# renaudbedard/raytracing-in-one-weekend

Hardware: AMD Instinct MI355X
Metric: Msamples/s, 486-sphere cover scene 1920x1080 8-bounce (higher is better)
Workload: dtype f32

## Files before the change

### include/rtow.h

```cpp
#ifndef RTOW_H
#define RTOW_H

#include <stddef.h>
#include <stdint.h>

#ifdef __cplusplus
extern "C" {
#endif

#if defined(_WIN32)
#define RTOW_API __declspec(dllexport)
#else
#define RTOW_API __attribute__((visibility("default")))
#endif

#define RTOW_API_VERSION 12

typedef enum RtowResult {
    RTOW_SUCCESS = 0,
    RTOW_ERROR_INVALID_VALUE = 1,
    RTOW_ERROR_MEMORY_ALLOCATION = 2,
    RTOW_ERROR_NO_DEVICE = 3,
    RTOW_ERROR_NO_SCENE = 4,
    RTOW_ERROR_UNSUPPORTED = 5,
// ... 102 lines not shown
    int32_t sceneInLds;
    uint64_t sceneBytesDevice;
    uint64_t hitSpillBytes;
    int32_t hitListCapacity;
    int32_t wideCodes;
    int32_t thresholdSet;
    int32_t schedulerTune[9];
} RtowSceneInfo;


typedef struct RtowView {
    RtowFloat3 origin;
    RtowFloat3 lowerLeftCorner;
    RtowFloat3 horizontal, vertical;
    RtowFloat3 forward, up, right;
    float lensRadius;
} RtowView;

typedef enum RtowRngPolicy { RTOW_RNG_REFERENCE = 0, RTOW_RNG_PER_SAMPLE = 1, RTOW_RNG_PER_SAMPLE_XOROSHIRO = 2 } RtowRngPolicy;

typedef enum RtowCubemapChannelType { RTOW_CUBEMAP_UNSIGNED_BYTE = 0, RTOW_CUBEMAP_SIGNED_HALF = 1 } RtowCubemapChannelType;
typedef struct RtowCubemapDesc {
    int32_t faceWidth, faceHeight;
    int32_t channelType;
    int32_t pixelStride;
    const void* faces;
} RtowCubemapDesc;

typedef struct RtowBlueNoiseDesc {
    uint32_t rowStride, textureCount;
    const void* texels;
} RtowBlueNoiseDesc;
typedef struct RtowStbNoiseDesc {
    uint32_t rowStride, textureCount;
    const void* scalar;
    const void* vector2;
    const void* cosineUnitVector3;
    const void* unitVector2;
    const void* unitVector3;
} RtowStbNoiseDesc;

typedef struct RtowEnvironment {
    int32_t skyType;
    RtowFloat3 skyBottomColor;
    RtowFloat3 skyTopColor;
} RtowEnvironment;

typedef struct RtowSampleParams {
    RtowFloat2 size;
    int32_t sliceOffset;
    int32_t sliceDivider;
    uint32_t seed;
    RtowView view;
    RtowEnvironment environment;
    uint32_t sampleCountRange[2];
    int32_t traceDepth;
    int32_t subPixelJitter;
    int32_t noiseColor;
    RtowFloat2 sampleCountWeightExtrema;
    int32_t diagnosticsStride;
    int32_t noiseTextureIndex;
    int32_t rngPolicy;
} RtowSampleParams;

typedef struct RtowAccumBuffers {
    float* color;
    float* normal;
    float* albedo;
    float* sampleCountWeight;
} RtowAccumBuffers;

typedef struct RtowContext_t* RtowContext;

typedef void (*RtowLogCallback)(int32_t level, const char* tag, const char* message, void* userData);

typedef enum RtowContextFlags {
    RTOW_CONTEXT_EXACT_TIES_ALWAYS = 1u << 0,
    RTOW_CONTEXT_EXACT_TIES_NEVER = 1u << 1,
    RTOW_CONTEXT_REFERENCE_DIAGNOSTICS = 1u << 2,
    RTOW_CONTEXT_NO_CAMERA_RAY_LISTS = 1u << 3,
    RTOW_CONTEXT_NO_CHUNK_ORDER = 1u << 4,
    RTOW_CONTEXT_FORCE_WIDE_CODES = 1u << 5,
    RTOW_CONTEXT_NO_CHAIN_FUSION = 1u << 7,
    RTOW_CONTEXT_NO_THRESHOLD_TUNING = 1u << 6
} RtowContextFlags;

typedef struct RtowContextOptions {
    int32_t deviceOrdinal;
    RtowLogCallback logCallback;
    void* logCallbackData;
    int32_t logCallbackLevel;
    uint32_t flags;
    int32_t ldsSceneBudgetBytes;
    int32_t schedulerTune[9];
    int32_t hitListCapacity;
    int32_t sliceBlockThreads;
} RtowContextOptions;

RTOW_API int rtowGetApiVersion(void);
RTOW_API const char* rtowErrorString(int result);

RTOW_API int rtowCreateContext(const RtowContextOptions* options, RtowContext* outContext);
RTOW_API int rtowDestroyContext(RtowContext context);

RTOW_API int rtowUploadScene(RtowContext context, const RtowSceneDesc* scene);
RTOW_API int rtowGetSceneInfo(RtowContext context, RtowSceneInfo* outInfo);

RTOW_API int rtowUploadSkyCubemap(RtowContext context, const RtowCubemapDesc* cubemap);

RTOW_API int rtowUploadBlueNoise(RtowContext context, const RtowBlueNoiseDesc* noise);
RTOW_API int rtowUploadStbNoise(RtowContext context, const RtowStbNoiseDesc* noise);

RTOW_API int rtowSampleBatch(RtowContext context, const RtowSampleParams* params,
                             const RtowAccumBuffers* in, const RtowAccumBuffers* out,
                             void* diagnostics, const volatile uint8_t* cancel);

RTOW_API int rtowSampleBatchDevice(RtowContext context, const RtowSampleParams* params,
                                   const RtowAccumBuffers* in, const RtowAccumBuffers* out,
                                   void* diagnostics, void* stream, const volatile uint8_t* cancel);

RTOW_API int rtowSampleBatchChainDevice(RtowContext context, int32_t count, const RtowSampleParams* params ,
                                        const RtowAccumBuffers* in, const RtowAccumBuffers* out,
                                        void* const* diagnostics , void* stream, const volatile uint8_t* cancel);

typedef struct RtowAdaptiveFeed {
    const RtowFloat2* extremaIn;
    RtowFloat2* extremaOut;
    int32_t lag;
    int32_t reserved;
} RtowAdaptiveFeed;

RTOW_API int rtowSampleBatchChainAdaptiveDevice(RtowContext context, int32_t count, const RtowSampleParams* params ,
                                                const RtowAccumBuffers* in, const RtowAccumBuffers* out,
                                                void* const* diagnostics , const RtowAdaptiveFeed* feed,
                                                void* stream, const volatile uint8_t* cancel);

RTOW_API int rtowSampleBatchGroupDevice(RtowContext context, int32_t count, const RtowSampleParams* params ,
                                        const RtowAccumBuffers* in, const RtowAccumBuffers* outs ,
                                        void* const* diagnostics , void* stream, const volatile uint8_t* cancel);

RTOW_API int rtowSampleBatchChain(RtowContext context, int32_t count, const RtowSampleParams* params ,
                                  const RtowAccumBuffers* in, const RtowAccumBuffers* out,
                                  void* const* diagnostics , const volatile uint8_t* cancel);

RTOW_API int rtowRegisterHostBuffer(RtowContext context, void* pointer, size_t sizeInBytes);
RTOW_API int rtowUnregisterHostBuffer(RtowContext context, void* pointer);

RTOW_API int rtowProbeNearestHit(RtowContext context, const RtowFloat3* origin, const RtowFloat3* direction, float time, float* distance, int32_t* entityIndex);

typedef struct RtowRay {
    RtowFloat3 origin;  float time;
    RtowFloat3 direction; float pad;
} RtowRay;

typedef struct RtowHitBuffers {
    float*   distance;
    int32_t* entityIndex;
    float*   normal;
} RtowHitBuffers;

RTOW_API int rtowTraceRaysDevice(RtowContext context, int32_t count, const RtowRay* rays ,
                                 const RtowHitBuffers* hits, void* stream);

typedef struct RtowTraceViewParams {
    int32_t width, height;
    RtowView view;
// ... 102 lines not shown
```

### raytracing-in-one-weekend_amd/abi.py

```python
import ctypes as C

RTOW_API_VERSION = 12

RTOW_SUCCESS = 0
RTOW_ERROR_INVALID_VALUE = 1
RTOW_ERROR_MEMORY_ALLOCATION = 2
RTOW_ERROR_NO_DEVICE = 3
RTOW_ERROR_NO_SCENE = 4
RTOW_ERROR_UNSUPPORTED = 5
RTOW_ERROR_LAUNCH_FAILURE = 6
RTOW_ERROR_CANCELLED = 7
RTOW_ERROR_CAPACITY = 8
RTOW_ERROR_INTERNAL = 99

ENTITY_NONE, ENTITY_SPHERE, ENTITY_RECT, ENTITY_BOX, ENTITY_TRIANGLE = range(5)
MATERIAL_STANDARD, MATERIAL_DIELECTRIC, MATERIAL_PROBABILISTIC_VOLUME = range(3)
TEXTURE_NONE, TEXTURE_CONSTANT, TEXTURE_CHECKER_PATTERN, TEXTURE_PERLIN_NOISE, TEXTURE_IMAGE, TEXTURE_CONSTANT_SCALAR = range(6)
SKY_NONE, SKY_GRADIENT, SKY_CUBEMAP = range(3)
NOISE_WHITE, NOISE_BLUE, NOISE_SPATIOTEMPORAL_BLUE = range(3)
MEMCPY_HOST_TO_HOST, MEMCPY_HOST_TO_DEVICE, MEMCPY_DEVICE_TO_HOST, MEMCPY_DEVICE_TO_DEVICE = range(4)


class Float2(C.Structure):
    _fields_ = [("x", C.c_float), ("y", C.c_float)]
# ... 18 lines not shown
                ("scalarValueChannel", C.c_int32), ("imageIndex", C.c_int32)]


class Image(C.Structure):
    _fields_ = [("width", C.c_int32), ("height", C.c_int32), ("pixelStride", C.c_int32), ("pixels", C.c_void_p)]


class Material(C.Structure):
    _fields_ = [("type", C.c_int32), ("albedo", Texture), ("glossiness", Texture), ("emission", Texture),
                ("metallic", Texture), ("parameter", C.c_float)]


class Entity(C.Structure):
    _fields_ = [("type", C.c_int32), ("moving", C.c_int32), ("rotation", Float4), ("position", Float3),
                ("destinationOffset", Float3), ("timeRange", Float2), ("materialIndex", C.c_int32),
                ("size", Float3), ("contentIndex", C.c_int32)]


class Triangle(C.Structure):
    _fields_ = [("data", Float3 * 3), ("normals", Float3 * 3), ("textureCoordinates", Float2 * 3)]


class SceneDesc(C.Structure):
    _fields_ = [("entities", C.POINTER(Entity)), ("entityCount", C.c_int32),
                ("materials", C.POINTER(Material)), ("materialCount", C.c_int32),
                ("maxBvhDepth", C.c_int32), ("triangles", C.POINTER(Triangle)), ("triangleCount", C.c_int32),
                ("images", C.POINTER(Image)), ("imageCount", C.c_int32)]


class SceneInfo(C.Structure):
    _fields_ = [("entityCount", C.c_int32), ("materialCount", C.c_int32), ("bvhNodeCount", C.c_int32),
                ("bvhDepth", C.c_int32), ("ldsBytesScene", C.c_int32), ("sceneInLds", C.c_int32),
                ("sceneBytesDevice", C.c_uint64), ("hitSpillBytes", C.c_uint64), ("hitListCapacity", C.c_int32), ("wideCodes", C.c_int32),
                ("thresholdSet", C.c_int32), ("schedulerTune", C.c_int32 * 9)]


class View(C.Structure):
    _fields_ = [("origin", Float3), ("lowerLeftCorner", Float3), ("horizontal", Float3), ("vertical", Float3),
                ("forward", Float3), ("up", Float3), ("right", Float3), ("lensRadius", C.c_float)]


CUBEMAP_UNSIGNED_BYTE, CUBEMAP_SIGNED_HALF = 0, 1
RNG_REFERENCE, RNG_PER_SAMPLE, RNG_PER_SAMPLE_XOROSHIRO = 0, 1, 2


class CubemapDesc(C.Structure):
    _fields_ = [("faceWidth", C.c_int32), ("faceHeight", C.c_int32), ("channelType", C.c_int32), ("pixelStride", C.c_int32),
                ("faces", C.c_void_p)]


class BlueNoiseDesc(C.Structure):
    _fields_ = [("rowStride", C.c_uint32), ("textureCount", C.c_uint32), ("texels", C.c_void_p)]


class StbNoiseDesc(C.Structure):
    _fields_ = [("rowStride", C.c_uint32), ("textureCount", C.c_uint32), ("scalar", C.c_void_p), ("vector2", C.c_void_p),
                ("cosineUnitVector3", C.c_void_p), ("unitVector2", C.c_void_p), ("unitVector3", C.c_void_p)]


class Environment(C.Structure):
    _fields_ = [("skyType", C.c_int32), ("skyBottomColor", Float3), ("skyTopColor", Float3)]


class SampleParams(C.Structure):
    _fields_ = [("size", Float2), ("sliceOffset", C.c_int32), ("sliceDivider", C.c_int32), ("seed", C.c_uint32),
                ("view", View), ("environment", Environment), ("sampleCountRange", C.c_uint32 * 2),
                ("traceDepth", C.c_int32), ("subPixelJitter", C.c_int32), ("noiseColor", C.c_int32),
                ("sampleCountWeightExtrema", Float2), ("diagnosticsStride", C.c_int32), ("noiseTextureIndex", C.c_int32),
                ("rngPolicy", C.c_int32)]


class AccumBuffers(C.Structure):
    _fields_ = [("color", C.c_void_p), ("normal", C.c_void_p), ("albedo", C.c_void_p),
                ("sampleCountWeight", C.c_void_p)]


class AdaptiveFeed(C.Structure):
    _fields_ = [("extremaIn", C.c_void_p), ("extremaOut", C.c_void_p), ("lag", C.c_int32), ("reserved", C.c_int32)]


LogCallback = C.CFUNCTYPE(None, C.c_int32, C.c_char_p, C.c_char_p, C.c_void_p)


CONTEXT_EXACT_TIES_ALWAYS, CONTEXT_EXACT_TIES_NEVER, CONTEXT_REFERENCE_DIAGNOSTICS, CONTEXT_NO_CAMERA_RAY_LISTS, CONTEXT_NO_CHUNK_ORDER, CONTEXT_FORCE_WIDE_CODES, CONTEXT_NO_THRESHOLD_TUNING, CONTEXT_NO_CHAIN_FUSION = 1, 2, 4, 8, 16, 32, 64, 128
GATHER_COLOR, GATHER_NORMAL, GATHER_ALBEDO, GATHER_SAMPLE_COUNT_WEIGHT, GATHER_ALL, GATHER_NO_BATCH_WAIT, GATHER_LOOPBACK = 1, 2, 4, 8, 15, 16, 32


class ContextOptions(C.Structure):
    _fields_ = [("deviceOrdinal", C.c_int32), ("logCallback", LogCallback), ("logCallbackData", C.c_void_p),
                ("logCallbackLevel", C.c_int32), ("flags", C.c_uint32), ("ldsSceneBudgetBytes", C.c_int32), ("schedulerTune", C.c_int32 * 9),
                ("hitListCapacity", C.c_int32), ("sliceBlockThreads", C.c_int32)]


class CommId(C.Structure):
    _fields_ = [("bytes", C.c_char * 128)]


class HybridPlan(C.Structure):
    _fields_ = [("tileCount", C.c_int32), ("groupCount", C.c_int32), ("tile", C.c_int32), ("group", C.c_int32),
                ("sliceOffset", C.c_int32), ("sliceDivider", C.c_int32), ("samples", C.c_uint32), ("seed", C.c_uint32)]


class Metrics(C.Structure):
    _fields_ = [("totalRayCount", C.c_int32), ("totalSamples", C.c_int32), ("sampleCountWeightExtrema", Float2),
                ("sampleCountExtrema", C.c_int32 * 2), ("totalRayCount64", C.c_int64), ("totalSamples64", C.c_int64)]


class CombineParams(C.Structure):
    _fields_ = [("width", C.c_int32), ("height", C.c_int32), ("debugMode", C.c_int32), ("ldrAlbedo", C.c_int32)]


RTOW_DENOISE_DEMODULATE_ALBEDO = 1
DENOISE_DEFAULT_ITERATIONS = 5
DENOISE_DEFAULT_NORMAL_SHARPNESS = 4
DENOISE_DEFAULT_COLOR_SIGMA = 0.5
DENOISE_DEFAULT_ALBEDO_SIGMA = 0.5
DENOISE_DEFAULT_FLAGS = RTOW_DENOISE_DEMODULATE_ALBEDO


class DenoiseParams(C.Structure):
    _fields_ = [("width", C.c_int32), ("height", C.c_int32), ("iterations", C.c_int32), ("normalSharpness", C.c_int32),
                ("colorSigma", C.c_float), ("albedoSigma", C.c_float), ("flags", C.c_int32), ("reserved", C.c_int32)]


class Ray(C.Structure):
    _fields_ = [("origin", Float3), ("time", C.c_float), ("direction", Float3), ("pad", C.c_float)]


RAY_DTYPE = [("origin", "<f4", (3,)), ("time", "<f4"), ("direction", "<f4", (3,)), ("pad", "<f4")]


class HitBuffers(C.Structure):
    _fields_ = [("distance", C.c_void_p), ("entityIndex", C.c_void_p), ("normal", C.c_void_p)]


class TraceViewParams(C.Structure):
    _fields_ = [("width", C.c_int32), ("height", C.c_int32), ("view", View), ("time", C.c_float), ("reserved", C.c_int32)]


def denoise_scratch_bytes(width, height):
    return int(width) * int(height) * 12


EXPORTED_SYMBOLS = [
    "rtowGetApiVersion", "rtowErrorString", "rtowCreateContext", "rtowDestroyContext", "rtowUploadScene",
    "rtowUploadSkyCubemap", "rtowUploadBlueNoise", "rtowUploadStbNoise", "rtowGetSceneInfo", "rtowSampleBatch", "rtowSampleBatchDevice", "rtowGetLastSampleKernelMs",
    "rtowReduceMetricsDevice", "rtowCombineDevice", "rtowFinalizeDevice", "rtowAddAccumDevice", "rtowDeviceAlloc", "rtowDeviceFree",
    "rtowDeviceCopy", "rtowDeviceMemset", "rtowSynchronize", "rtowGetBatchStatus", "rtowRegisterHostBuffer", "rtowUnregisterHostBuffer",
    "rtowSampleBatchChainDevice", "rtowSampleBatchChain", "rtowCommSetLibraryPath", "rtowCommGetUniqueId", "rtowCommInit", "rtowCommDestroy", "rtowGatherRowsDevice",
    "rtowHybridPlan", "rtowExchangeAccumDevice", "rtowSampleBatchGroupDevice",
    "rtowCombineFinalizeDevice", "rtowReduceMetricsDeviceAsync", "rtowProbeNearestHit", "rtowSampleBatchChainAdaptiveDevice",
    "rtowDenoiseDevice", "rtowTraceRaysDevice", "rtowTraceViewDevice",
]
```

### raytracing-in-one-weekend_amd/csrc/rtow_api.hip

```cpp
#include <hip/hip_runtime.h>

#include <algorithm>
#include <atomic>
#include <cfloat>
#include <chrono>
#include <cstdio>
#include <cstring>
#include <mutex>
#include <string>
#include <thread>
#include <vector>

#include "../../include/rtow.h"
#include "rtow_context.h"

#ifndef RTOW_GROUP_SLOT_BLOCK
#define RTOW_GROUP_SLOT_BLOCK 4
#endif
static constexpr unsigned kGroupSlotBlock = RTOW_GROUP_SLOT_BLOCK;
#ifndef RTOW_PIXEL_GATE
#define RTOW_PIXEL_GATE 1
#endif
#ifndef RTOW_URGENT_RAYS_PER_SAMPLE
#define RTOW_URGENT_RAYS_PER_SAMPLE 18.0f
// ... 852 lines not shown
    void* pinnedDevice = nullptr;
    ok = ok && hipHostGetDevicePointer(&pinnedDevice, pinned, 0) == hipSuccess;
    if (!ok) { if (pinned) (void)hipHostFree(pinned); rtowDestroyContext(ctx); return RTOW_ERROR_MEMORY_ALLOCATION; }
    ctx->hCancel = (volatile uint32_t*)pinned;
    ctx->hMetricsRecord = (volatile RtowMetrics*)((uint8_t*)pinned + 64);
    ctx->dMetricsRecord = (RtowMetrics*)((uint8_t*)pinnedDevice + 64);
    ctx->hCancel[0] = 0u;
    ctx->hCancel[1] = 0u;
    ctx->hCancel[2] = 0u;
    ctx->hCancel[3] = 0u;
    logf(ctx, 4, "rtow", "context on device %d (%s, %d CUs)", ordinal, prop.gcnArchName, ctx->cuCount);
    if (ctx->flags & RTOW_CONTEXT_NO_CHAIN_FUSION) {
        ctx->chainFusion = false;
    } else {
        unsigned pairs = 0, stale = 0, timeouts = 0;
        hipError_t le = hipSuccess;
        for (int attempt = 0; attempt < 2; attempt++) {
            le = runXcdCoherenceLitmus(ctx->cuCount, ctx->stream, &pairs, &stale, &timeouts);
            if (le != hipSuccess || stale != 0 || (pairs > 0 && timeouts == 0)) break;
            logf(ctx, 3, "rtow", "same-XCD hand-over litmus inconclusive (%u pairs, %u timeouts): %s", pairs, timeouts, attempt == 0 ? "once more" : "giving up");
        }
        ctx->chainFusion = le == hipSuccess && pairs > 0 && stale == 0 && timeouts == 0;
        if (le != hipSuccess) (void)hipGetLastError();
        logf(ctx, ctx->chainFusion ? 4 : 3, "rtow", "same-XCD hand-over litmus: %u pairs, %u stale dwords, %u timeouts%s", pairs, stale, timeouts,
             ctx->chainFusion ? "" : stale ? " - unsafe here: chained batches will run one launch per batch" : " - inconclusive: chained batches will run one launch per batch");
    }
    *outContext = ctx;
    return RTOW_SUCCESS;
}

RTOW_API int rtowDestroyContext(RtowContext ctx)
{
    if (!ctx) return RTOW_ERROR_INVALID_VALUE;
    (void)hipSetDevice(ctx->device);
    if (ctx->stream) (void)hipStreamSynchronize(ctx->stream);
    if (ctx->dScene) (void)hipFree(ctx->dScene);
    if (ctx->dEntityOfPrim) (void)hipFree(ctx->dEntityOfPrim);
    if (ctx->dWorkCounter) (void)hipFree(ctx->dWorkCounter);
    if (ctx->dChunkCost) { (void)hipFree(ctx->dChunkCost); (void)hipFree(ctx->dChunkOrder); (void)hipFree(ctx->dPixelCost); (void)hipFree(ctx->dTicketMap); }
    if (ctx->dChunkDone) (void)hipFree(ctx->dChunkDone);
    if (ctx->dXcdState) (void)hipFree(ctx->dXcdState);
    if (ctx->dChainBatches) (void)hipFree(ctx->dChainBatches);
    if (ctx->dPixCand) (void)hipFree(ctx->dPixCand);
    if (ctx->dCubemap) (void)hipFree(ctx->dCubemap);
    if (ctx->dBlueNoise) (void)hipFree(ctx->dBlueNoise);
    if (ctx->dStbNoise) (void)hipFree(ctx->dStbNoise);
    if (ctx->dTexBlob) (void)hipFree(ctx->dTexBlob);
    if (ctx->dRefTree) (void)hipFree(ctx->dRefTree);
    if (ctx->dHitSpill) (void)hipFree(ctx->dHitSpill);
    if (ctx->dUnitRecords) (void)hipFree(ctx->dUnitRecords);
    if (ctx->dPartials) (void)hipFree(ctx->dPartials);
    if (ctx->dExtremaPartials) (void)hipFree(ctx->dExtremaPartials);
    if (ctx->dExtremaKeys) (void)hipFree(ctx->dExtremaKeys);
    if (ctx->dByteThresholds) (void)hipFree(ctx->dByteThresholds);
    dropThresholdTuning(ctx);
    if (ctx->dProbeSink) (void)hipFree(ctx->dProbeSink);
    if (ctx->dTieRedo) (void)hipFree(ctx->dTieRedo);
    if (ctx->dTieBits) (void)hipFree(ctx->dTieBits);
    if (ctx->dTieInputs) (void)hipFree(ctx->dTieInputs);
    if (ctx->dHistSpill) (void)hipFree(ctx->dHistSpill);
    if (ctx->dRedoSpill) (void)hipFree(ctx->dRedoSpill);
    if (ctx->hCancel) (void)hipHostFree((void*)ctx->hCancel);
    if (ctx->dColor) { (void)hipFree(ctx->dColor); (void)hipFree(ctx->dNormal); (void)hipFree(ctx->dAlbedo); (void)hipFree(ctx->dScw); }
    if (ctx->dDiag) (void)hipFree(ctx->dDiag);
    releaseComm(ctx);
    for (const RtowContext_t::HostRange& r : ctx->hostRanges) (void)hipHostUnregister(r.base);
    ctx->hostRanges.clear();
    if (ctx->evStart) (void)hipEventDestroy(ctx->evStart);
    if (ctx->evStop) (void)hipEventDestroy(ctx->evStop);
    if (ctx->evBatchDone) (void)hipEventDestroy(ctx->evBatchDone);
    if (ctx->evMetricsDone) (void)hipEventDestroy(ctx->evMetricsDone);
    if (ctx->stream) (void)hipStreamDestroy(ctx->stream);
    delete ctx;
    return RTOW_SUCCESS;
}

RTOW_API int rtowUploadScene(RtowContext ctx, const RtowSceneDesc* scene)
{
    if (!ctx || !scene) return RTOW_ERROR_INVALID_VALUE;
    std::lock_guard<std::mutex> lock(ctx->mu);
    HIP_TRY(ctx, hipSetDevice(ctx->device), RTOW_ERROR_NO_DEVICE);
    CompiledScene compiled;
    std::string err;
    const int rc = compileScene(scene, RTOW_STACK_CAPACITY, &compiled, &err);
    if (rc != RTOW_SUCCESS) {
        logf(ctx, 2, "scene", "%s", err.c_str());
        return rc;
    }
    HIP_TRY(ctx, hipDeviceSynchronize(), RTOW_ERROR_LAUNCH_FAILURE);
    RTOW_TRY(growDevice(ctx, ctx->dSceneCapacity, compiled.blob.size(), {devBuf(ctx->dScene, compiled.blob.size())}));
    HIP_TRY(ctx, hipMemcpy(ctx->dScene, compiled.blob.data(), compiled.blob.size(), hipMemcpyHostToDevice), RTOW_ERROR_LAUNCH_FAILURE);
    if (!compiled.entityOfPrim.empty()) {
        const size_t n = compiled.entityOfPrim.size();
        RTOW_TRY(growDevice(ctx, ctx->entityOfPrimCapacity, n, {devBuf(ctx->dEntityOfPrim, n * sizeof(int32_t))}));
        HIP_TRY(ctx, hipMemcpy(ctx->dEntityOfPrim, compiled.entityOfPrim.data(), n * sizeof(int32_t), hipMemcpyHostToDevice), RTOW_ERROR_LAUNCH_FAILURE);
    }
    if (!compiled.texBlob.empty()) {
        RTOW_TRY(growDevice(ctx, ctx->texBlobCapacity, compiled.texBlob.size(), {devBuf(ctx->dTexBlob, compiled.texBlob.size())}));
        HIP_TRY(ctx, hipMemcpy(ctx->dTexBlob, compiled.texBlob.data(), compiled.texBlob.size(), hipMemcpyHostToDevice), RTOW_ERROR_LAUNCH_FAILURE);
        compiled.texBlob.clear();
        compiled.texBlob.shrink_to_fit();
    }
    if (ctx->flags & RTOW_CONTEXT_REFERENCE_DIAGNOSTICS) {
        if (compiled.refTreeDepth > 62) { logf(ctx, 2, "scene", "RTOW_CONTEXT_REFERENCE_DIAGNOSTICS supports MaxBvhDepth <= 62"); return RTOW_ERROR_CAPACITY; }
        RTOW_TRY(growDevice(ctx, ctx->refTreeCapacity, compiled.refTree.size(), {devBuf(ctx->dRefTree, compiled.refTree.size())}));
        HIP_TRY(ctx, hipMemcpy(ctx->dRefTree, compiled.refTree.data(), compiled.refTree.size(), hipMemcpyHostToDevice), RTOW_ERROR_LAUNCH_FAILURE);
    }
    compiled.refTree.clear();
    compiled.refTree.shrink_to_fit();
    HIP_TRY(ctx, launchPrepareMaterials(ctx->dScene, compiled.layout, ctx->stream), RTOW_ERROR_LAUNCH_FAILURE);
    HIP_TRY(ctx, launchPrepareEntities(ctx->dScene, compiled.layout, ctx->stream), RTOW_ERROR_LAUNCH_FAILURE);
    HIP_TRY(ctx, hipStreamSynchronize(ctx->stream), RTOW_ERROR_LAUNCH_FAILURE);
    if (compiled.layout.sceneKind >= SCENE_KIND_GENERAL && compiled.entityCount > 0)
        HIP_TRY(ctx, hipMemcpy(compiled.blob.data() + compiled.layout.primOffset, ctx->dScene + compiled.layout.primOffset, (size_t)compiled.entityCount * sizeof(GpuPrim), hipMemcpyDeviceToHost),
                RTOW_ERROR_LAUNCH_FAILURE);
    if (ctx->flags & (RTOW_CONTEXT_EXACT_TIES_ALWAYS | RTOW_CONTEXT_EXACT_TIES_NEVER)) {
        const bool volumes = compiled.layout.sceneKind == SCENE_KIND_VOLUMES || compiled.layout.sceneKind == SCENE_KIND_VOLUMES_TEXTURED;
        if (!volumes) compiled.layout.exactTies = (ctx->flags & RTOW_CONTEXT_EXACT_TIES_ALWAYS) ? 1u : 0u;
    }
    {
        const int rc = sizeHitSpill(ctx, compiled.layout.sceneKind, compiled.layout.exactTies != 0, compiled.entityCount);
        if (rc != RTOW_SUCCESS) return rc;
    }
    const bool wide = compiled.entityCount > 65535 || compiled.layout.nodeCount > 65535u || (ctx->flags & RTOW_CONTEXT_FORCE_WIDE_CODES) != 0;
    ctx->wideCodes = wide;
    if (!ctx->userTune) {
        const int* base = kThresholdFamilies[compiled.layout.sceneKind <= SCENE_KIND_SPHERES_MOTION ? 0 : 1];
        for (int k = 0; k < 9; k++) ctx->tune[k] = base[k];
    } else if (ctx->userSliceDefault) {
        ctx->tune[8] = 16;
    }
    std::lock_guard<std::mutex> sceneLock(ctx->sceneMu);
    ctx->scene = std::move(compiled);
    ctx->ldsPlan = planLds(wide, ctx->scene.layout, 0u, ctx->ldsSceneBudget);
    ctx->ldsSceneBytes = ctx->ldsPlan.sceneBytes;
    ctx->ldsNodeCount = ctx->ldsPlan.nodeCount;
    ctx->haveScene = true;
    ctx->triWatchOff = false;
    ctx->hCancel[3] = 0u;
    ctx->sceneSerial++;
    ctx->orderValid = false;
    dropThresholdTuning(ctx);
    ctx->sppSinceUpload = 0;
    ctx->sceneSignatureNow = sceneSignature(ctx->scene, wide);
    if (!ctx->userTune && !(ctx->flags & RTOW_CONTEXT_NO_THRESHOLD_TUNING))
        for (const RtowContext_t::TuneCacheEntry& e : ctx->tuneCache)
            if (e.signature == ctx->sceneSignatureNow) {
                candidateThresholds(e.winner, ctx->tune, 8);
                ctx->tunedCandidate = e.winner;
                ctx->tunedScene = ctx->sceneSerial;
            }
    logf(ctx, 4, "scene", "%d entities, %u BVH nodes, depth %u, %u bytes (%u in LDS)%s", ctx->scene.entityCount, ctx->scene.layout.nodeCount,
         ctx->scene.layout.bvhDepth, ctx->scene.layout.totalBytes, ctx->ldsSceneBytes,
         ctx->scene.layout.exactTies ? ", exact-tie kernels" : "");
    return RTOW_SUCCESS;
}

RTOW_API int rtowUploadSkyCubemap(RtowContext ctx, const RtowCubemapDesc* cubemap)
{
    if (!ctx) return RTOW_ERROR_INVALID_VALUE;
    std::lock_guard<std::mutex> lock(ctx->mu);
    HIP_TRY(ctx, hipSetDevice(ctx->device), RTOW_ERROR_NO_DEVICE);
    if (!cubemap || !cubemap->faces) {
        HIP_TRY(ctx, hipDeviceSynchronize(), RTOW_ERROR_LAUNCH_FAILURE);
        if (ctx->dCubemap) (void)hipFree(ctx->dCubemap);
        ctx->dCubemap = nullptr;
        ctx->cubemapCapacity = 0;
// ... 483 lines not shown
```

### raytracing-in-one-weekend_amd/csrc/rtow_bvh.cpp

```cpp
#include "rtow_bvh.h"
#include "rtow_reforder.h"

#include <algorithm>
#include <cfloat>
#include <cmath>
#include <cstring>
#include <numeric>
#include <queue>

namespace rtow {

namespace {

struct Box {
    float lo[3], hi[3];
    void reset() { for (int a = 0; a < 3; a++) { lo[a] = FLT_MAX; hi[a] = -FLT_MAX; } }
    void grow(const Box& b) { for (int a = 0; a < 3; a++) { lo[a] = std::min(lo[a], b.lo[a]); hi[a] = std::max(hi[a], b.hi[a]); } }
    double area() const
    {
        const double dx = (double)hi[0] - lo[0], dy = (double)hi[1] - lo[1], dz = (double)hi[2] - lo[2];
        return 2.0 * (dx * dy + dy * dz + dz * dx);
    }
};

// ... 51 lines not shown

        const int self = (int)nodes.size();
        nodes.push_back(TmpNode{});
        Box b0, b1;
        const int c0 = build(idx, begin, begin + bestSplit, depthLeft - 1, depth + 1, &b0);
        const int c1 = build(idx, begin + bestSplit, end, depthLeft - 1, depth + 1, &b1);
        nodes[self].box[0] = b0; nodes[self].box[1] = b1;
        nodes[self].child[0] = c0; nodes[self].child[1] = c1;
        *outBox = b0;
        outBox->grow(b1);
        return self;
    }

    int buildBinned(std::vector<int>& idx, int begin, int end, int depthLeft, int depth, long long cap, Box* outBox)
    {
        const int n = end - begin;
        float clo[3] = {FLT_MAX, FLT_MAX, FLT_MAX}, chi[3] = {-FLT_MAX, -FLT_MAX, -FLT_MAX};
        for (int i = begin; i < end; i++)
            for (int a = 0; a < 3; a++) { const float c = centroid[a][idx[i]]; clo[a] = std::min(clo[a], c); chi[a] = std::max(chi[a], c); }
        double bestCost = DBL_MAX;
        int bestAxis = -1, bestBin = -1;
        for (int axis = 0; axis < 3; axis++) {
            const float ext = chi[axis] - clo[axis];
            if (!(ext > 0)) continue;
            const float scale = (float)kBins / ext;
            Box bb[kBins];
            int cnt[kBins] = {0};
            for (int b = 0; b < kBins; b++) bb[b].reset();
            for (int i = begin; i < end; i++) {
                int b = (int)((centroid[axis][idx[i]] - clo[axis]) * scale);
                b = b < 0 ? 0 : b >= kBins ? kBins - 1 : b;
                cnt[b]++;
                bb[b].grow(primBox[idx[i]]);
            }
            double rArea[kBins];
            int rCnt[kBins];
            Box acc;
            acc.reset();
            int c = 0;
            for (int b = kBins - 1; b >= 1; b--) { if (cnt[b]) acc.grow(bb[b]); c += cnt[b]; rArea[b] = c ? acc.area() : 0.0; rCnt[b] = c; }
            acc.reset();
            c = 0;
            for (int b = 1; b < kBins; b++) {
                if (cnt[b - 1]) acc.grow(bb[b - 1]);
                c += cnt[b - 1];
                if (c == 0 || rCnt[b] == 0 || c > cap || rCnt[b] > cap) continue;
                const double cost = acc.area() * c + rArea[b] * rCnt[b];
                if (cost < bestCost) { bestCost = cost; bestAxis = axis; bestBin = b; }
            }
        }
        int mid;
        if (bestAxis >= 0) {
            const float scale = (float)kBins / (chi[bestAxis] - clo[bestAxis]);
            const std::vector<float>& cc = centroid[bestAxis];
            const float lo = clo[bestAxis];
            const int bin = bestBin;
            int* first = idx.data() + begin;
            int* split = std::partition(first, idx.data() + end, [&](int p) {
                int b = (int)((cc[p] - lo) * scale);
                b = b < 0 ? 0 : b >= kBins ? kBins - 1 : b;
                return b < bin;
            });
            mid = begin + (int)(split - first);
        } else {
            int axis = 0;
            for (int a = 1; a < 3; a++) if (chi[a] - clo[a] > chi[axis] - clo[axis]) axis = a;
            const std::vector<float>& cc = centroid[axis];
            mid = begin + n / 2;
            std::nth_element(idx.begin() + begin, idx.begin() + mid, idx.begin() + end, [&cc](int a, int b) { return cc[a] < cc[b] || (cc[a] == cc[b] && a < b); });
        }
        const int self = (int)nodes.size();
        nodes.push_back(TmpNode{});
        Box b0, b1;
        const int c0 = build(idx, begin, mid, depthLeft - 1, depth + 1, &b0);
        const int c1 = build(idx, mid, end, depthLeft - 1, depth + 1, &b1);
        nodes[self].box[0] = b0; nodes[self].box[1] = b1;
        nodes[self].child[0] = c0; nodes[self].child[1] = c1;
        *outBox = b0;
        outBox->grow(b1);
        return self;
    }
};

float texColor(const RtowTexture& t, int c)
{
    switch (t.type) {
        case RTOW_TEXTURE_CONSTANT: return c == 0 ? t.mainColor.x : c == 1 ? t.mainColor.y : t.mainColor.z;
        case RTOW_TEXTURE_CONSTANT_SCALAR: return t.parameter;
    }
    return 0.0f;
}
float texScalar(const RtowTexture& t)
{
    switch (t.type) {
        case RTOW_TEXTURE_CONSTANT: return texColor(t, t.scalarValueChannel);
        case RTOW_TEXTURE_CONSTANT_SCALAR: return t.parameter;
    }
    return 0.0f;
}
bool texSupported(const RtowTexture& t)
{
    return t.type == RTOW_TEXTURE_NONE || t.type == RTOW_TEXTURE_CONSTANT || t.type == RTOW_TEXTURE_CONSTANT_SCALAR || t.type == RTOW_TEXTURE_IMAGE;
}
GpuTexture packTexture(const RtowTexture& t)
{
    GpuTexture g{};
    g.type = t.type;
    g.image = t.type == RTOW_TEXTURE_IMAGE ? t.imageIndex : -1;
    g.channel = t.scalarValueChannel;
    g.parameter = t.parameter;
    g.mainColor[0] = t.mainColor.x; g.mainColor[1] = t.mainColor.y; g.mainColor[2] = t.mainColor.z;
    return g;
}
bool almostOne(float v) { return std::fabs(1.0f - v) < 1e-6f; }

uint32_t align16(uint32_t v) { return (v + 15u) & ~15u; }

void setBoxes(GpuNode& g, const Box& b0, const Box& b1)
{
    g.lox[0] = b0.lo[0]; g.lox[1] = b1.lo[0]; g.loy[0] = b0.lo[1]; g.loy[1] = b1.lo[1]; g.loz[0] = b0.lo[2]; g.loz[1] = b1.lo[2];
    g.hix[0] = b0.hi[0]; g.hix[1] = b1.hi[0]; g.hiy[0] = b0.hi[1]; g.hiy[1] = b1.hi[1]; g.hiz[0] = b0.hi[2]; g.hiz[1] = b1.hi[2];
}

}

int compileScene(const RtowSceneDesc* desc, int maxDepth, CompiledScene* out, std::string* err)
{
    if (!desc || !out || !desc->entities || !desc->materials || desc->entityCount <= 0 || desc->materialCount <= 0) {
        *err = "null or empty scene description";
        return RTOW_ERROR_INVALID_VALUE;
    }
    const int n = desc->entityCount;
    if (n > (1 << 23) || desc->materialCount > 32767) {
        *err = "scene exceeds 8388608 entities or 32767 materials (30-bit hit codes / 32-bit blob offsets, 15-bit path-history codes)";
        return RTOW_ERROR_CAPACITY;
    }
    if (maxDepth <= 0) maxDepth = RTOW_DEFAULT_MAX_BVH_DEPTH;
    if (maxDepth > RTOW_STACK_CAPACITY) maxDepth = RTOW_STACK_CAPACITY;
    if ((1LL << std::min(maxDepth, 30)) < n) {
        *err = "maxBvhDepth too small for the entity count";
        return RTOW_ERROR_CAPACITY;
    }

    std::vector<GpuMaterial> mats(desc->materialCount);
    std::vector<uint32_t> matClass(desc->materialCount);
    bool hasVolumes = false, hasImageTextures = false;
    for (int i = 0; i < desc->materialCount; i++) {
        const RtowMaterial& m = desc->materials[i];
        if (m.type != RTOW_MATERIAL_STANDARD && m.type != RTOW_MATERIAL_DIELECTRIC && m.type != RTOW_MATERIAL_PROBABILISTIC_VOLUME) {
            *err = "unknown material type";
            return RTOW_ERROR_INVALID_VALUE;
        }
        hasVolumes |= m.type == RTOW_MATERIAL_PROBABILISTIC_VOLUME;
        if (!texSupported(m.albedo) || !texSupported(m.glossiness) || !texSupported(m.emission) || !texSupported(m.metallic)) {
            *err = "texture type not built (CheckerPattern / PerlinNoise are dead code in the reference)";
            return RTOW_ERROR_UNSUPPORTED;
        }
        bool textured = false;
        for (const RtowTexture* t : {&m.albedo, &m.glossiness, &m.emission, &m.metallic}) {
            if (t->type != RTOW_TEXTURE_IMAGE) continue;
            textured = true;
            if (t->imageIndex >= desc->imageCount || (t->imageIndex >= 0 && !desc->images)) {
                *err = "imageIndex out of range";
                return RTOW_ERROR_INVALID_VALUE;
            }
            if (t->scalarValueChannel < 0 || t->scalarValueChannel > 2) {
                *err = "scalarValueChannel out of range";
                return RTOW_ERROR_INVALID_VALUE;
            }
        }
        hasImageTextures |= textured;
        GpuMaterial g{};
        for (int c = 0; c < 3; c++) { g.albedo[c] = texColor(m.albedo, c); g.emission[c] = texColor(m.emission, c); }
        g.type = m.type;
        g.metallic = texScalar(m.metallic);
        g.glossiness = texScalar(m.glossiness);
        g.parameter = (m.type == RTOW_MATERIAL_DIELECTRIC || m.type == RTOW_MATERIAL_PROBABILISTIC_VOLUME) ? m.parameter : 0.0f;
        g.flags = 0;
        bool spec = false;
        if (m.type == RTOW_MATERIAL_DIELECTRIC) spec = true;
        else if (m.type == RTOW_MATERIAL_STANDARD)
            spec = m.metallic.type == RTOW_TEXTURE_CONSTANT && almostOne(m.metallic.mainColor.x) && almostOne(m.metallic.mainColor.y) &&
                    almostOne(m.metallic.mainColor.z) && m.glossiness.type == RTOW_TEXTURE_CONSTANT && almostOne(m.glossiness.mainColor.x) &&
                    almostOne(m.glossiness.mainColor.y) && almostOne(m.glossiness.mainColor.z);
        if (spec) g.flags |= MAT_FLAG_PERFECT_SPECULAR;
        if (textured) g.flags |= MAT_FLAG_TEXTURED;
        mats[i] = g;
        matClass[i] = m.type == RTOW_MATERIAL_PROBABILISTIC_VOLUME ? MAT_CLASS_VOLUME : m.type == RTOW_MATERIAL_DIELECTRIC ? MAT_CLASS_DIELECTRIC
                      : (g.glossiness == 0.0f && g.metallic == 0.0f && !textured) ? MAT_CLASS_LAMBERT : MAT_CLASS_GENERAL;
    }

    std::vector<GpuSphere> spheres(n);
    std::vector<GpuMotion> motion(n);
    std::vector<GpuPrim> prims;
    std::vector<float> cullBoxes;
    std::vector<uint32_t> matIndex(n);
    bool hasMotion = false, general = hasVolumes || hasImageTextures;
    for (int i = 0; i < n; i++) {
        const RtowEntity& e = desc->entities[i];
        const bool identity = e.rotation.x == 0.0f && e.rotation.y == 0.0f && e.rotation.z == 0.0f && e.rotation.w == 1.0f;
        if (e.type != RTOW_ENTITY_SPHERE || !identity) general = true;
    }
    if (general) prims.resize(n);
    cullBoxes.assign((size_t)n * 8, 0.0f);
    Builder b;
    b.primBox.resize(n);
    for (int a = 0; a < 3; a++) b.centroid[a].resize(n);
    for (int i = 0; i < n; i++) {
        const RtowEntity& e = desc->entities[i];
// ... 76 lines not shown
            }
            cullBoxes[i * 8 + 0] = cl[0]; cullBoxes[i * 8 + 1] = cl[1]; cullBoxes[i * 8 + 2] = cl[2];
            cullBoxes[i * 8 + 4] = ch[0]; cullBoxes[i * 8 + 5] = ch[1]; cullBoxes[i * 8 + 6] = ch[2];
        }
        for (int a = 0; a < 3; a++) {
            const float ext = bx.hi[a] - bx.lo[a];
            const float pad = 1e-5f * std::max(std::max(std::fabs(bx.lo[a]), std::fabs(bx.hi[a])), 1.0f) + 1e-5f * ext;
            b.centroid[a][i] = 0.5f * (bx.lo[a] + bx.hi[a]);
            bx.lo[a] -= pad;
            bx.hi[a] += pad;
        }
        b.primBox[i] = bx;

        if (general) {
            GpuPrim g{};
            if (e.type == RTOW_ENTITY_TRIANGLE) {
                memcpy(g.q, &desc->triangles[e.contentIndex], sizeof(RtowTriangle));
                g.q[24] = e.rotation.x; g.q[25] = e.rotation.y; g.q[26] = e.rotation.z; g.q[27] = e.rotation.w;
            } else {
                g.q[0] = e.rotation.x; g.q[1] = e.rotation.y; g.q[2] = e.rotation.z; g.q[3] = e.rotation.w;
                g.q[8] = e.position.x; g.q[9] = e.position.y; g.q[10] = e.position.z;
                const int32_t mv = e.moving ? 1 : 0;
                memcpy(&g.q[11], &mv, 4);
                g.q[12] = e.destinationOffset.x; g.q[13] = e.destinationOffset.y; g.q[14] = e.destinationOffset.z; g.q[15] = e.timeRange.x;
                g.q[16] = e.timeRange.y;
                if (e.type == RTOW_ENTITY_SPHERE) {
                    g.q[20] = e.size.x;
                } else if (e.type == RTOW_ENTITY_RECT) {
                    g.q[20] = -e.size.x / 2; g.q[21] = -e.size.y / 2; g.q[22] = e.size.x / 2; g.q[23] = e.size.y / 2;
                } else {
                    g.q[20] = e.size.x / 2; g.q[21] = e.size.y / 2; g.q[22] = e.size.z / 2;
                    g.q[23] = 1 / g.q[20]; g.q[24] = 1 / g.q[21]; g.q[25] = 1 / g.q[22];
                }
            }
            prims[i] = g;
        }
    }

    std::vector<float> guardBoxes;
    std::vector<RefTreeNode> refTree;
    const std::vector<uint32_t> ranks = referenceLeafRanks(cullBoxes, n, desc->maxBvhDepth > 0 ? desc->maxBvhDepth : 32 , &guardBoxes, &refTree);
    out->refTree.assign(reinterpret_cast<const uint8_t*>(refTree.data()), reinterpret_cast<const uint8_t*>(refTree.data()) + refTree.size() * sizeof(RefTreeNode));
    out->refTreeDepth = desc->maxBvhDepth > 0 ? desc->maxBvhDepth : 32;
    for (int i = 0; i < n; i++) {
        bool wider = false;
        for (int a = 0; a < 3; a++) wider |= guardBoxes[(size_t)i * 8 + a] < cullBoxes[(size_t)i * 8 + a] || guardBoxes[(size_t)i * 8 + 4 + a] > cullBoxes[(size_t)i * 8 + 4 + a];
        if (!wider) continue;
        Box& bx = b.primBox[i];
        for (int a = 0; a < 3; a++) {
            const float lo = guardBoxes[(size_t)i * 8 + a], hi = guardBoxes[(size_t)i * 8 + 4 + a];
            const float pad = 1e-5f * std::max(std::max(std::fabs(lo), std::fabs(hi)), 1.0f) + 1e-5f * (hi - lo);
            bx.lo[a] = std::min(bx.lo[a], lo - pad);
            bx.hi[a] = std::max(bx.hi[a], hi + pad);
            b.centroid[a][i] = 0.5f * (bx.lo[a] + bx.hi[a]);
        }
    }
    cullBoxes = guardBoxes;

    bool allTriangles = general;
    for (int i = 0; i < n && allTriangles; i++) allTriangles = desc->entities[i].type == RTOW_ENTITY_TRIANGLE;
    const bool triKind = allTriangles && !hasVolumes;
    std::vector<int> placeOf;
    auto leafPlace = [&](int entity) { return triKind && !placeOf.empty() ? placeOf[entity] : entity; };
    std::vector<uint32_t> ranksInLeafOrder(triKind ? n : 0);
    out->entityOfPrim.clear();

    std::vector<int> idx(n);
    std::iota(idx.begin(), idx.end(), 0);
    Box rootBox;
    std::vector<GpuNode> gnodes;
    int depthSeen = 0;
    if (n == 1) {
        GpuNode g{};
        Box empty;
        empty.reset();
        Box only;
        for (int a = 0; a < 3; a++) { only.lo[a] = cullBoxes[a]; only.hi[a] = cullBoxes[4 + a]; }
        setBoxes(g, only, empty);
        g.child0 = ~0; g.child1 = ~0;
        gnodes.push_back(g);
        depthSeen = 1;
    } else {
        b.nodes.reserve(n);
        const int root = b.build(idx, 0, n, maxDepth, 0, &rootBox);
        depthSeen = b.maxDepthSeen;
        if (triKind) {
            placeOf.resize(n);
            for (int k = 0; k < n; k++) placeOf[idx[k]] = k;
        }
        constexpr size_t kBreadthFirstNodes = 2048;
        std::vector<int> newIndex(b.nodes.size(), -1);
        std::vector<int> bfs;
        bfs.reserve(b.nodes.size());
        std::queue<int> q;
        q.push(root);
        while (!q.empty() && bfs.size() < kBreadthFirstNodes) {
            const int t = q.front();
            q.pop();
            newIndex[t] = (int)bfs.size();
            bfs.push_back(t);
            for (int c = 0; c < 2; c++) if (b.nodes[t].child[c] >= 0) q.push(b.nodes[t].child[c]);
        }
        std::vector<int> dfs;
        while (!q.empty()) {
            dfs.push_back(q.front());
            q.pop();
            while (!dfs.empty()) {
                const int t = dfs.back();
                dfs.pop_back();
                newIndex[t] = (int)bfs.size();
                bfs.push_back(t);
                for (int c = 1; c >= 0; c--) if (b.nodes[t].child[c] >= 0) dfs.push_back(b.nodes[t].child[c]);
            }
        }
        gnodes.resize(bfs.size());
        for (size_t i = 0; i < bfs.size(); i++) {
            const TmpNode& t = b.nodes[bfs[i]];
            GpuNode g{};
            Box cb[2] = {t.box[0], t.box[1]};
            for (int c = 0; c < 2; c++)
                if (t.child[c] < 0) {
                    const float* e = &cullBoxes[(size_t)(~t.child[c]) * 8];
                    for (int a = 0; a < 3; a++) { cb[c].lo[a] = e[a]; cb[c].hi[a] = e[4 + a]; }
                }
            setBoxes(g, cb[0], cb[1]);
            g.child0 = t.child[0] >= 0 ? newIndex[t.child[0]] : ~leafPlace(~t.child[0]);
            g.child1 = t.child[1] >= 0 ? newIndex[t.child[1]] : ~leafPlace(~t.child[1]);
            gnodes[i] = g;
        }
    }
    if (triKind && n > 1) {
        auto permute = [&](auto& v, size_t per) {
            if (v.empty()) return;
            auto w = v;
            for (int i = 0; i < n; i++) std::copy(w.begin() + (size_t)i * per, w.begin() + (size_t)(i + 1) * per, v.begin() + (size_t)placeOf[i] * per);
        };
        permute(spheres, 1); permute(motion, 1); permute(prims, 1); permute(cullBoxes, 8); permute(matIndex, 1);
        std::vector<uint32_t> r = ranks;
        for (int i = 0; i < n; i++) ranksInLeafOrder[placeOf[i]] = r[i];
        out->entityOfPrim.assign(n, 0);
        for (int i = 0; i < n; i++) out->entityOfPrim[placeOf[i]] = i;
    }
    {
        const uint64_t bytes = (uint64_t)gnodes.size() * sizeof(GpuNode) + (uint64_t)n * (sizeof(GpuSphere) + (hasMotion ? sizeof(GpuMotion) : 0) + (general ? sizeof(GpuPrim) : 0) + (hasVolumes ? 32u : 0u) + (triKind ? sizeof(GpuTriHot) + sizeof(GpuTriCold) : 0) + 8u) +
                               (uint64_t)mats.size() * sizeof(GpuMaterial) + 256u;
        if (bytes >= 0xfff00000ull) {
            *err = "scene image exceeds 4 GiB";
            return RTOW_ERROR_CAPACITY;
        }
    }

    SceneLayout L{};
    uint32_t off = 0;
    L.nodeOffset = off; L.nodeCount = (uint32_t)gnodes.size(); off = align16(off + L.nodeCount * (uint32_t)sizeof(GpuNode));
    L.sphereOffset = off; L.sphereCount = (uint32_t)n; off = align16(off + (uint32_t)n * (uint32_t)sizeof(GpuSphere));
    L.hasMotion = hasMotion ? 1u : 0u;
    if (hasMotion) {
        bool first = true, same = true;
        uint32_t t0 = 0, t1 = 0;
        for (int i = 0; i < n && same; i++) {
            const RtowEntity& e = desc->entities[i];
            if (!e.moving) continue;
            uint32_t a, b;
            memcpy(&a, &e.timeRange.x, 4); memcpy(&b, &e.timeRange.y, 4);
            if (first) { t0 = a; t1 = b; first = false; }
            else same = a == t0 && b == t1;
        }
        if (same && !first) { L.commonTimeRange = 1u; memcpy(&L.commonT0, &t0, 4); memcpy(&L.commonT1, &t1, 4); }
// ... 124 lines not shown
```

### raytracing-in-one-weekend_amd/csrc/rtow_bvh.h

```cpp
#pragma once
#include <stdint.h>

#include <string>
#include <vector>

#include "../../include/rtow.h"
#include "rtow_scene.h"

#define RTOW_STACK_CAPACITY 24
#define RTOW_DEFAULT_MAX_BVH_DEPTH 24

namespace rtow {

struct CompiledScene {
    std::vector<uint8_t> blob;
    SceneLayout layout;
    int entityCount = 0;
    int materialCount = 0;
    std::vector<uint8_t> texBlob;
    TexLayout texLayout{};
    std::vector<uint8_t> refTree;
    int refTreeDepth = 0;
    std::vector<int32_t> entityOfPrim;
};

int compileScene(const RtowSceneDesc* desc, int maxDepth, CompiledScene* out, std::string* err);

}
```

Baseline: 9594.

## Optimize BVH with SAH-driven subtree reinsertion after top-down build

Adds a post-build optimization pass that repeatedly detaches subtrees and reinserts them where the sum of node surface areas drops, using a branch-and-bound priority search capped by the original depth limit. Leaf order is then recomputed from the new tree. The goal is a tighter BVH that needs fewer node visits per ray during traversal. It adds host-side scene compile time, applies only to scenes at or below the binned-build threshold, and can be turned off with a new context flag.

```diff
diff --git a/include/rtow.h b/include/rtow.h
--- a/include/rtow.h
+++ b/include/rtow.h
@@ -208,6 +208,7 @@
     RTOW_CONTEXT_NO_CHUNK_ORDER = 1u << 4,
     RTOW_CONTEXT_FORCE_WIDE_CODES = 1u << 5,
     RTOW_CONTEXT_NO_CHAIN_FUSION = 1u << 7,
+    RTOW_CONTEXT_TOP_DOWN_TREE = 1u << 8,
     RTOW_CONTEXT_NO_THRESHOLD_TUNING = 1u << 6
 } RtowContextFlags;
 
diff --git a/raytracing-in-one-weekend_amd/abi.py b/raytracing-in-one-weekend_amd/abi.py
--- a/raytracing-in-one-weekend_amd/abi.py
+++ b/raytracing-in-one-weekend_amd/abi.py
@@ -124,7 +124,7 @@
 LogCallback = C.CFUNCTYPE(None, C.c_int32, C.c_char_p, C.c_char_p, C.c_void_p)
 
 
-CONTEXT_EXACT_TIES_ALWAYS, CONTEXT_EXACT_TIES_NEVER, CONTEXT_REFERENCE_DIAGNOSTICS, CONTEXT_NO_CAMERA_RAY_LISTS, CONTEXT_NO_CHUNK_ORDER, CONTEXT_FORCE_WIDE_CODES, CONTEXT_NO_THRESHOLD_TUNING, CONTEXT_NO_CHAIN_FUSION = 1, 2, 4, 8, 16, 32, 64, 128
+CONTEXT_EXACT_TIES_ALWAYS, CONTEXT_EXACT_TIES_NEVER, CONTEXT_REFERENCE_DIAGNOSTICS, CONTEXT_NO_CAMERA_RAY_LISTS, CONTEXT_NO_CHUNK_ORDER, CONTEXT_FORCE_WIDE_CODES, CONTEXT_NO_THRESHOLD_TUNING, CONTEXT_NO_CHAIN_FUSION, CONTEXT_TOP_DOWN_TREE = 1, 2, 4, 8, 16, 32, 64, 128, 256
 GATHER_COLOR, GATHER_NORMAL, GATHER_ALBEDO, GATHER_SAMPLE_COUNT_WEIGHT, GATHER_ALL, GATHER_NO_BATCH_WAIT, GATHER_LOOPBACK = 1, 2, 4, 8, 15, 16, 32
 
 
diff --git a/raytracing-in-one-weekend_amd/csrc/rtow_api.hip b/raytracing-in-one-weekend_amd/csrc/rtow_api.hip
--- a/raytracing-in-one-weekend_amd/csrc/rtow_api.hip
+++ b/raytracing-in-one-weekend_amd/csrc/rtow_api.hip
@@ -958,7 +958,7 @@
     HIP_TRY(ctx, hipSetDevice(ctx->device), RTOW_ERROR_NO_DEVICE);
     CompiledScene compiled;
     std::string err;
-    const int rc = compileScene(scene, RTOW_STACK_CAPACITY, &compiled, &err);
+    const int rc = compileScene(scene, RTOW_STACK_CAPACITY, &compiled, &err, (ctx->flags & RTOW_CONTEXT_TOP_DOWN_TREE) != 0);
     if (rc != RTOW_SUCCESS) {
         logf(ctx, 2, "scene", "%s", err.c_str());
         return rc;
diff --git a/raytracing-in-one-weekend_amd/csrc/rtow_bvh.cpp b/raytracing-in-one-weekend_amd/csrc/rtow_bvh.cpp
--- a/raytracing-in-one-weekend_amd/csrc/rtow_bvh.cpp
+++ b/raytracing-in-one-weekend_amd/csrc/rtow_bvh.cpp
@@ -157,6 +157,155 @@
     }
 };
 
+struct Reinserter {
+    std::vector<TmpNode>& nodes;
+    const std::vector<Box>& primBox;
+    int root;
+    const int depthLimit;
+    std::vector<int> parent;
+    std::vector<int> leafParent;
+    std::vector<int> height;
+
+    struct Entry {
+        double induced;
+        int code, depth;
+        bool operator<(const Entry& o) const { return induced > o.induced || (induced == o.induced && code > o.code); }
+    };
+    std::vector<Entry> heap;
+
+    Reinserter(std::vector<TmpNode>& nodes_, const std::vector<Box>& primBox_, int root_, int depthLimit_)
+        : nodes(nodes_), primBox(primBox_), root(root_), depthLimit(depthLimit_), parent(nodes_.size(), -1), leafParent(primBox_.size(), -1), height(nodes_.size(), 0)
+    {
+        for (int i = 0; i < (int)nodes.size(); i++)
+            for (int s = 0; s < 2; s++) setParent(nodes[i].child[s], i);
+        for (int i = (int)nodes.size() - 1; i >= 0; i--) height[i] = 1 + std::max(heightOf(nodes[i].child[0]), heightOf(nodes[i].child[1]));
+    }
+
+    Box boxOf(int code) const
+    {
+        if (code < 0) return primBox[~code];
+        Box b = nodes[code].box[0];
+        b.grow(nodes[code].box[1]);
+        return b;
+    }
+    int heightOf(int code) const { return code < 0 ? 0 : height[code]; }
+    int parentOf(int code) const { return code < 0 ? leafParent[~code] : parent[code]; }
+    void setParent(int code, int p) { if (code < 0) leafParent[~code] = p; else parent[code] = p; }
+    static Box merged(Box a, const Box& b) { a.grow(b); return a; }
+
+    void refitUp(int p)
+    {
+        while (p >= 0) {
+            height[p] = 1 + std::max(heightOf(nodes[p].child[0]), heightOf(nodes[p].child[1]));
+            const int q = parent[p];
+            if (q >= 0) nodes[q].box[nodes[q].child[0] == p ? 0 : 1] = boxOf(p);
+            p = q;
+        }
+    }
+
+    double objective() const
+    {
+        double sum = 0.0;
+        for (int i = 0; i < (int)nodes.size(); i++) sum += boxOf(i).area();
+        return sum;
+    }
+
+    void detach(int N, int s)
+    {
+        const int T = nodes[N].child[1 - s], P = parent[N];
+        if (P < 0) {
+            root = T;
+            parent[T] = -1;
+            return;
+        }
+        const int ps = nodes[P].child[0] == N ? 0 : 1;
+        nodes[P].child[ps] = T;
+        nodes[P].box[ps] = nodes[N].box[1 - s];
+        setParent(T, P);
+        refitUp(P);
+    }
+
+    void attach(int N, int s, int X)
+    {
+        const int Q = parentOf(X);
+        nodes[N].child[1 - s] = X;
+        nodes[N].box[1 - s] = boxOf(X);
+        parent[N] = Q;
+        if (Q < 0) root = N;
+        else nodes[Q].child[nodes[Q].child[0] == X ? 0 : 1] = N;
+        setParent(X, N);
+        refitUp(N);
+    }
+
+    double costNextTo(int X, const Box& sBox) const
+    {
+        int chain[RTOW_STACK_CAPACITY + 8], len = 0;
+        for (int a = parentOf(X); a >= 0 && len < RTOW_STACK_CAPACITY + 8; a = parent[a]) chain[len++] = a;
+        double induced = 0.0;
+        for (int k = len - 1; k >= 0; k--) {
+            const Box bx = boxOf(chain[k]);
+            induced = (induced + merged(bx, sBox).area()) - bx.area();
+        }
+        return induced + merged(boxOf(X), sBox).area();
+    }
+
+    bool reinsert(int N, int s)
+    {
+        const int S = nodes[N].child[s], T = nodes[N].child[1 - s];
+        if (parent[N] < 0 && T < 0) return false;
+        const Box sBox = boxOf(S);
+        const double sArea = sBox.area();
+        const int hS = heightOf(S);
+        detach(N, s);
+        const double oldCost = costNextTo(T, sBox);
+        double best = oldCost - 1e-9 * oldCost;
+        int bestX = T;
+        heap.clear();
+        heap.push_back(Entry{0.0, root, 0});
+        while (!heap.empty()) {
+            std::pop_heap(heap.begin(), heap.end());
+            const Entry e = heap.back();
+            heap.pop_back();
+            if (e.induced + sArea >= best) break;
+            const Box bx = boxOf(e.code);
+            const double total = e.induced + merged(bx, sBox).area();
+            if (total < best && e.code != T && e.depth + 1 + std::max(hS, heightOf(e.code)) <= depthLimit) { best = total; bestX = e.code; }
+            if (e.code >= 0) {
+                const double below = total - bx.area();
+                if (below + sArea < best && e.depth + 2 + hS <= depthLimit)
+                    for (int c = 0; c < 2; c++) {
+                        heap.push_back(Entry{below, nodes[e.code].child[c], e.depth + 1});
+                        std::push_heap(heap.begin(), heap.end());
+                    }
+            }
+        }
+        attach(N, s, bestX);
+        return bestX != T;
+    }
+
+    void run()
+    {
+        const int m = (int)nodes.size();
+        std::vector<int> order(m);
+        std::vector<double> area(m);
+        double before = objective();
+        for (int pass = 0; pass < kMaxPasses; pass++) {
+            for (int i = 0; i < m; i++) { order[i] = i; area[i] = boxOf(i).area(); }
+            std::sort(order.begin(), order.end(), [&area](int a, int b) { return area[a] > area[b] || (area[a] == area[b] && a < b); });
+            bool moved = false;
+            for (int k = 0; k < m; k++)
+                for (int s = 0; s < 2; s++) moved |= reinsert(order[k], s);
+            const double after = objective();
+            const bool done = !moved || !(before - after >= kMinGain * before);
+            before = after;
+            if (done) break;
+        }
+    }
+
+    static constexpr int kMaxPasses = 8;
+    static constexpr double kMinGain = 1e-3;
+};
+
 float texColor(const RtowTexture& t, int c)
 {
     switch (t.type) {
@@ -199,7 +348,7 @@
 
 }
 
-int compileScene(const RtowSceneDesc* desc, int maxDepth, CompiledScene* out, std::string* err)
+int compileScene(const RtowSceneDesc* desc, int maxDepth, CompiledScene* out, std::string* err, bool keepTopDownTree)
 {
     if (!desc || !out || !desc->entities || !desc->materials || desc->entityCount <= 0 || desc->materialCount <= 0) {
         *err = "null or empty scene description";
@@ -442,8 +591,23 @@
         depthSeen = 1;
     } else {
         b.nodes.reserve(n);
-        const int root = b.build(idx, 0, n, maxDepth, 0, &rootBox);
+        int root = b.build(idx, 0, n, maxDepth, 0, &rootBox);
         depthSeen = b.maxDepthSeen;
+        if (!keepTopDownTree && n > 2 && n <= kBinnedAbove) {
+            Reinserter r(b.nodes, b.primBox, root, std::min(b.maxDepthSeen, maxDepth));
+            r.run();
+            root = r.root;
+            depthSeen = r.height[root];
+            int k = 0;
+            std::vector<int> stack{root};
+            while (!stack.empty()) {
+                const int t = stack.back();
+                stack.pop_back();
+                if (t < 0) { idx[k++] = ~t; continue; }
+                stack.push_back(b.nodes[t].child[1]);
+                stack.push_back(b.nodes[t].child[0]);
+            }
+        }
         if (triKind) {
             placeOf.resize(n);
             for (int k = 0; k < n; k++) placeOf[idx[k]] = k;
diff --git a/raytracing-in-one-weekend_amd/csrc/rtow_bvh.h b/raytracing-in-one-weekend_amd/csrc/rtow_bvh.h
--- a/raytracing-in-one-weekend_amd/csrc/rtow_bvh.h
+++ b/raytracing-in-one-weekend_amd/csrc/rtow_bvh.h
@@ -24,6 +24,6 @@
     std::vector<int32_t> entityOfPrim;
 };
 
-int compileScene(const RtowSceneDesc* desc, int maxDepth, CompiledScene* out, std::string* err);
+int compileScene(const RtowSceneDesc* desc, int maxDepth, CompiledScene* out, std::string* err, bool keepTopDownTree = false);
 
 }
```

Result: no change. 9591 (median of 2 runs) (-0.0%).
